# alpc91/SGRL

Measured on AMD Instinct MI355X. Metric: env-steps/sec (whole node) + SET-actor fwd us/step, 3d_walker mix @8192 envs/GPU, higher is better.
Workload: dtype f64 (dynamics) / f32 (SET actor, obs); 1 GPU; 3D_Walker++ 8 variants x 1024 envs per GPU (config 3), random U(-1,1) actions, auto-reset, SET actor forward on every step, random-init weights; envs_per_gpu=8192, obs_max_len=287, action_max_len=21, replay_gather=none (single rank)

## Files before the change

### include/sgrl.h

```cpp
#ifndef SGRL_H
#define SGRL_H

#include <stdint.h>

#ifdef __cplusplus
extern "C" {
#endif

typedef struct sgrl_engine sgrl_engine;

enum {
  SGRL_OK = 0,
  SGRL_ERR_ARG = -1,
  SGRL_ERR_MODEL = -2,
  SGRL_ERR_HIP = -3,
  SGRL_ERR_LIMIT = -4
};

int sgrl_engine_create(int n_morph, const int32_t* const* ib, const int32_t* ib_len, const double* const* fb,
                       const int32_t* fb_len, const int32_t* morph_count, int obs_max_len, int action_max_len,
                       uint64_t seed, uint32_t env_id_base, int max_episode_steps, sgrl_engine** out);
void sgrl_engine_destroy(sgrl_engine* e);

int sgrl_num_envs(const sgrl_engine* e);
int sgrl_record_stride(const sgrl_engine* e);
int sgrl_lds_bytes(const sgrl_engine* e);
int sgrl_launch_groups(const sgrl_engine* e);
int sgrl_fixed_dim_groups(const sgrl_engine* e);
int sgrl_paired_envs(const sgrl_engine* e);

int sgrl_reset(sgrl_engine* e, float* obs, double* obs64, void* stream);

int sgrl_step(sgrl_engine* e, const float* actions, float* obs, float* reward, uint8_t* done, float* dist,
              uint8_t* truncated, double* obs64, double* reward64, int auto_reset, void* stream);

int sgrl_get_records(sgrl_engine* e, double* rec, int32_t* cnt);
int sgrl_set_records(sgrl_engine* e, const double* rec, const int32_t* cnt);
int sgrl_refresh(sgrl_engine* e, float* obs, double* obs64, void* stream);

int sgrl_time_steps(sgrl_engine* e, const float* actions, float* obs, float* reward, uint8_t* done, int reps,
                    void* stream, float* ms_out);

int sgrl_pack_transitions(const float* obs, int ld_obs, const float* action, int ld_act, const float* next_obs, int ld_next,
                          const float* reward, const float* done_f32, const uint8_t* done_u8, const uint8_t* store,
// ... 23 lines not shown
```

### sgrl_amd/_lib.py

```python
import ctypes
import os
import subprocess

_HERE = os.path.dirname(os.path.abspath(__file__))
LIB_PATH = os.environ.get("SGRL_HIP_LIB", os.path.join(_HERE, "libsgrl_hip.so"))
CSRC = os.path.join(_HERE, "csrc")
SOURCES = ["engine.hip", "set_actor.hip", "train_gemm.hip", "render.hip", "swat_actor.hip", "smp_actor.hip"]

_lib = None

_i32p = ctypes.POINTER(ctypes.c_int32)
_f64p = ctypes.POINTER(ctypes.c_double)


class SgrlError(RuntimeError):
    pass


HDR_DIM_FIELDS = (1, 2, 3, 4, 5, 6, 7, 8, 9, 16, 18)
LIGHT_NV = 12
ITAB_GLOBAL = set(x for x in os.environ.get("SGRL_BUILD_ITAB_GLOBAL", "humanoid").split(",") if x and x != "none")
PAIR_NV = {"walker": 15, "hopper": 15}


# ... 44 lines not shown
    hdrs = [os.path.join(CSRC, f) for f in os.listdir(CSRC) if f.endswith((".h", ".inc"))]
    hdrs += [os.path.join(_HERE, "..", "include", f) for f in ("sgrl.h", "sgrl_model.h", "sgrl_set.h", "sgrl_swat.h", "sgrl_smp.h", "sgrl_train.h", "sgrl_render.h")
             if os.path.exists(os.path.join(_HERE, "..", "include", f))]
    newest_hdr = max(os.path.getmtime(d) for d in hdrs)
    objdir = os.path.join(_HERE, "..", "build", "obj")
    os.makedirs(objdir, exist_ok=True)
    base = ["hipcc", "--offload-arch=gfx950", "-O3", "-std=c++17", "-fPIC", "-fno-slp-vectorize"]
    jobs = []
    for sname in SOURCES:
        src = os.path.join(CSRC, sname)
        if os.path.exists(src):
            jobs.append((os.path.join(objdir, sname.replace(".hip", ".o")), src, []))
    spec_src = os.path.join(CSRC, "step_spec.hip")
    for i, w, dims, itab in fams:
        members = ",".join("DimsFixed<%s>" % ",".join(str(x) for x in d) for d in dims)
        flags = ["-DSGRL_SPEC_ID=%d" % i, "-DSGRL_SPEC_WAVES=%d" % w, "-DSGRL_SPEC_FAMILY=" + members]
        if itab:
            flags.append("-DSGRL_ITAB_GLOBAL=1")
        tag = "%08x" % (hash_text(members + str(w) + ("g" if itab else "")) & 0xFFFFFFFF)
        jobs.append((os.path.join(objdir, "family_%d_%s.o" % (i, tag)), spec_src, flags))

    def compile_one(job):
        obj, src, flags = job
        if os.path.exists(obj) and os.path.getmtime(obj) >= max(newest_hdr, os.path.getmtime(src)):
            return False
        cmd = base + flags + ["-c", "-o", obj, src]
        if verbose:
            print(" ".join(cmd), flush=True)
        subprocess.check_call(cmd)
        return True

# ... 19 lines not shown
        raise SgrlError("HIP extension %s is missing: run `python -c 'import __graft_entry__ as g; g.build()'` "
                        "(no CPU fallback exists)" % LIB_PATH)
    import torch
    try:
        L = ctypes.CDLL(LIB_PATH)
    except OSError as e:
        raise SgrlError("cannot load %s: %s" % (LIB_PATH, e))
    L.sgrl_last_error.restype = ctypes.c_char_p
    L.sgrl_version.restype = ctypes.c_char_p
    L.sgrl_engine_create.restype = ctypes.c_int
    L.sgrl_engine_create.argtypes = [ctypes.c_int, ctypes.POINTER(_i32p), _i32p, ctypes.POINTER(_f64p), _i32p, _i32p,
                                     ctypes.c_int, ctypes.c_int, ctypes.c_uint64, ctypes.c_uint32, ctypes.c_int,
                                     ctypes.POINTER(ctypes.c_void_p)]
    L.sgrl_engine_destroy.argtypes = [ctypes.c_void_p]
    L.sgrl_engine_destroy.restype = None
    for name in ("sgrl_num_envs", "sgrl_record_stride", "sgrl_lds_bytes", "sgrl_launch_groups", "sgrl_fixed_dim_groups", "sgrl_paired_envs"):
        getattr(L, name).argtypes = [ctypes.c_void_p]
        getattr(L, name).restype = ctypes.c_int
    vp = ctypes.c_void_p
    L.sgrl_reset.argtypes = [vp, vp, vp, vp]
    L.sgrl_step.argtypes = [vp, vp, vp, vp, vp, vp, vp, vp, vp, ctypes.c_int, vp]
    L.sgrl_refresh.argtypes = [vp, vp, vp, vp]
    L.sgrl_get_records.argtypes = [vp, vp, vp]
    L.sgrl_set_records.argtypes = [vp, vp, vp]
    L.sgrl_time_steps.argtypes = [vp, vp, vp, vp, vp, ctypes.c_int, vp, ctypes.POINTER(ctypes.c_float)]
    ci = ctypes.c_int
    L.sgrl_pack_transitions.argtypes = [vp, ci, vp, ci, vp, ci, vp, vp, vp, vp, vp, vp, ci, ci, ci, vp]
    L.sgrl_ingest_rows.argtypes = [vp, ci, ci, ci, vp, vp, ci, vp]
    L.sgrl_ingest_block.argtypes = [vp, ci, ci, ci, vp, ci, vp, vp, vp, vp, vp]
    L.sgrl_round_record.argtypes = [vp, vp, vp, vp, vp, vp, vp, vp, vp, ci, ci, vp]
    L.sgrl_ingest_ws_words.argtypes = [ci]
    L.sgrl_ingest_ws_words.restype = ctypes.c_int64
    _lib = L
    return L


EXPORTS = ["sgrl_engine_create", "sgrl_engine_destroy", "sgrl_num_envs", "sgrl_record_stride", "sgrl_lds_bytes", "sgrl_launch_groups", "sgrl_fixed_dim_groups", "sgrl_paired_envs",
           "sgrl_reset", "sgrl_step", "sgrl_get_records", "sgrl_set_records", "sgrl_refresh", "sgrl_time_steps", "sgrl_pack_transitions", "sgrl_round_record", "sgrl_ingest_rows", "sgrl_ingest_block", "sgrl_ingest_ws_words",
           "sgrl_last_error", "sgrl_version"]


def check(rc, what):
    if rc != 0:
        raise SgrlError("%s failed (%d): %s" % (what, rc, lib().sgrl_last_error().decode()))
```

### sgrl_amd/csrc/engine.hip

```cpp
#include <hip/hip_runtime.h>

#include <algorithm>
#include <cstdio>
#include <cstdlib>
#include <cstring>
#include <string>
#include <vector>

#include "engine_kernel.h"
#include "stream_pick.h"

namespace {

thread_local std::string g_err;

int fail(int code, const std::string& msg) {
  g_err = msg;
  return code;
}
#define HIP_TRY(expr)                                                                              \
  do {                                                                                             \
    hipError_t _e = (expr);                                                                        \
    if (_e != hipSuccess)                                                                          \
      return fail(SGRL_ERR_HIP, std::string(#expr) + ": " + hipGetErrorString(_e));                \
// ... 18 lines not shown
  sgrl::HipWave w;
  const sgrl::StepIO io = make_io(a, out, env);
  sgrl::env_reset(w, m, o, S, I, io, true);
}

__global__ __launch_bounds__(64) void k_env_refresh(BatchArgs a, StepOut out) {
  const int env = __builtin_amdgcn_readfirstlane(a.block_env[blockIdx.x]);
  SgrlModelView m; sgrl::Layout o; double* S; int32_t* I;
  setup<DimsAny>(a, env, &m, &o, &S, &I);
  sgrl::HipWave w;
  const sgrl::StepIO io = make_io(a, out, env);
  sgrl::env_refresh(w, m, o, S, I, io);
}

typedef int (*SpecLaunch)(int, int, void*, const void*, const void*);
struct SpecFamily { int waves; int n; SpecLaunch launch; int itab_global; };
struct SpecMember { int family, slot; int dims[12]; };
}
#ifndef SGRL_NO_SPECS
#define SGRL_FAMILY(id, waves, n, itab) extern "C" int sgrl_spec_launch_##id(int, int, void*, const void*, const void*);
#define SGRL_MEMBER(...)
#include "spec_table.inc"
#undef SGRL_FAMILY
#undef SGRL_MEMBER
namespace {
const SpecFamily kFamilies[] = {
#define SGRL_FAMILY(id, waves, n, itab) {waves, n, sgrl_spec_launch_##id, itab},
#define SGRL_MEMBER(...)
#include "spec_table.inc"
#undef SGRL_FAMILY
#undef SGRL_MEMBER
};
const SpecMember kMembers[] = {
#define SGRL_FAMILY(id, waves, n, itab)
#define SGRL_MEMBER(fam, slot, ...) {fam, slot, {__VA_ARGS__}},
#include "spec_table.inc"
#undef SGRL_FAMILY
#undef SGRL_MEMBER
};
constexpr int kNumMembers = (int)(sizeof(kMembers) / sizeof(kMembers[0]));
}
#else
namespace {
const SpecFamily kFamilies[1] = {{0, 0, nullptr, 0}};
const SpecMember kMembers[1] = {{-1, -1, {0}}};
constexpr int kNumMembers = 0;
}
#endif
namespace {
int spec_for(const int32_t* hdr, int waves) {
  static const int fields[11] = {SGRL_H_NBODY, SGRL_H_NJNT, SGRL_H_NQ, SGRL_H_NV, SGRL_H_NU, SGRL_H_NGEOM, SGRL_H_NPAIR,
                                 SGRL_H_INTEGRATOR, SGRL_H_FRAME_SKIP, SGRL_H_MAX_ROWS, SGRL_H_SOLVER};
  for (int k = 0; k < kNumMembers; k++) {
    if (kFamilies[kMembers[k].family].waves != waves) continue;
    bool same = true;
    for (int f = 0; f < 11 && same; f++) same = kMembers[k].dims[f] == hdr[fields[f]];
    if (same) return k;
  }
  return -1;
}
}

struct sgrl_engine {
  int n_morph = 0, n_env = 0, stride = 0, lds_bytes = 0, scratch_stride = 0;
  int obs_max_len = 0, action_max_len = 0;
  std::vector<int32_t*> d_ib;
  std::vector<double*> d_fb;
  MorphDev* d_morphs = nullptr;
  int32_t* d_env_morph = nullptr;
  int32_t* d_block_env = nullptr;
  int32_t* d_step_env = nullptr;
  int32_t* d_step_mate = nullptr;
  int n_paired = 0;
  double* d_rec = nullptr;
  int32_t* d_cnt = nullptr;
  double* d_scratch = nullptr;
  BatchArgs args{};
  struct Group {
    int first = 0, count = 0, lds = 0; bool light = false; int spec = -1; hipStream_t stream = nullptr; hipEvent_t done = nullptr;
    int step_first = 0, step_count = 0, step_lds = 0;
  };
  std::vector<Group> groups;
  bool groups_checked = false;
  hipEvent_t fork = nullptr;
  std::vector<int> morph_lds;
};

namespace {
template <class K>
int launch_groups(sgrl_engine* e, K kernel_in, const StepOut& out, hipStream_t user, bool is_step = false) {
  auto pick = [&](const sgrl_engine::Group& g) { return (is_step && g.light) ? k_env_step_light : kernel_in; };
  auto launch = [&](const sgrl_engine::Group& g, const BatchArgs& a_in, hipStream_t st) -> int {
    const BatchArgs& a = a_in;
    if (is_step && g.spec >= 0) {
      BatchArgs b = a_in;
      b.block_env = e->d_step_env + g.step_first;
      b.block_mate = e->d_step_mate + g.step_first;
      const int rc = kFamilies[g.spec].launch(g.step_count, g.step_lds, st, &b, &out);
      return rc == 0 ? SGRL_OK : fail(SGRL_ERR_HIP, std::string("fixed-dimension step kernel launch failed: ") + hipGetErrorString((hipError_t)rc));
    }
    hipLaunchKernelGGL(pick(g), dim3(g.count), dim3(64), g.lds, st, a, out);
    return SGRL_OK;
  };
  if (e->groups.size() == 1) {
    const int rc = launch(e->groups[0], e->args, user);
    if (rc != SGRL_OK) return rc;
  } else {
    if (!e->groups_checked && sgrl_streams::enabled()) {
      hipStreamCaptureStatus cap = hipStreamCaptureStatusNone;
      (void)hipStreamIsCapturing(user, &cap);
      if (cap == hipStreamCaptureStatusNone) {
        std::vector<hipStream_t> taken;
        for (auto& g : e->groups) {
// ... 185 lines not shown
  if (host && hipMemcpyFromSymbol(host, HIP_SYMBOL(sgrl_engine_dev::g_phase_prof), sizeof(unsigned long long) * 16 * (size_t)n_env) != hipSuccess) return -2;
  if (reset) { static unsigned long long z[16 * 65536]; if (hipMemcpyToSymbol(HIP_SYMBOL(sgrl_engine_dev::g_phase_prof), z, sizeof(z)) != hipSuccess) return -3; }
  return 0;
}
#endif

void sgrl_engine_destroy(sgrl_engine* e) {
  if (!e) return;
  for (auto p : e->d_ib) if (p) (void)hipFree(p);
  for (auto p : e->d_fb) if (p) (void)hipFree(p);
  if (e->d_morphs) (void)hipFree(e->d_morphs);
  if (e->d_env_morph) (void)hipFree(e->d_env_morph);
  if (e->d_block_env) (void)hipFree(e->d_block_env);
  if (e->d_step_env) (void)hipFree(e->d_step_env);
  if (e->d_step_mate) (void)hipFree(e->d_step_mate);
  if (e->d_rec) (void)hipFree(e->d_rec);
  if (e->d_cnt) (void)hipFree(e->d_cnt);
  if (e->d_scratch) (void)hipFree(e->d_scratch);
  for (auto& g : e->groups) { if (g.stream) (void)hipStreamDestroy(g.stream); if (g.done) (void)hipEventDestroy(g.done); }
  if (e->fork) (void)hipEventDestroy(e->fork);
  delete e;
}

int sgrl_engine_create(int n_morph, const int32_t* const* ib, const int32_t* ib_len, const double* const* fb,
                       const int32_t* fb_len, const int32_t* morph_count, int obs_max_len, int action_max_len,
                       uint64_t seed, uint32_t env_id_base, int max_episode_steps, sgrl_engine** out) {
  if (!out) return fail(SGRL_ERR_ARG, "out is null");
  *out = nullptr;
  if (n_morph <= 0 || !ib || !ib_len || !fb || !fb_len || !morph_count) return fail(SGRL_ERR_ARG, "null or empty morphology list");
  int ndev = 0;
// ... 141 lines not shown
            e->n_paired += 2;
            i += 2;
          } else {
            step_env.push_back(order[i]); step_mate.push_back(-1);
            i++;
          }
        }
        if (const char* pad = getenv("SGRL_LDS_PAD")) { g.lds += atoi(pad); g.step_lds += atoi(pad); e->lds_bytes = std::max(e->lds_bytes, g.lds); }
        g.count = i - g.first;
        g.step_count = (int)step_env.size() - g.step_first;
        e->lds_bytes = std::max(e->lds_bytes, std::max(g.step_lds, g.lds));
        e->groups.push_back(g);
      }
      (void)hipMemcpy(e->d_step_env, step_env.data(), sizeof(int32_t) * step_env.size(), hipMemcpyHostToDevice);
      (void)hipMemcpy(e->d_step_mate, step_mate.data(), sizeof(int32_t) * step_mate.size(), hipMemcpyHostToDevice);
    } else {
      std::vector<int> cost(n_morph), cls(n_morph);
      bool light_batch = true;
      for (int k = 0; k < n_morph; k++) {
        cost[k] = ib[k][SGRL_H_NV];
        const int granule = 1280;
        int per_cu = (160 * 1024) / (((e->morph_lds[k] + granule - 1) / granule) * granule);
        cls[k] = per_cu > 8 ? 8 : per_cu;
        light_batch = light_batch && ib[k][SGRL_H_NV] <= kLightNv && per_cu >= kLightPerCu;
      }
      if (light_batch) for (int k = 0; k < n_morph; k++) cls[k] = kLightPerCu;
      std::stable_sort(order.begin(), order.end(), [&](int32_t x, int32_t y) {
        const int mx = env_morph[x], my = env_morph[y];
        if (cls[mx] != cls[my]) return cls[mx] < cls[my];
        return cost[mx] > cost[my];
// ... 54 lines not shown
  BatchArgs& a = e->args;
  a.morphs = e->d_morphs; a.env_morph = e->d_env_morph; a.block_env = e->d_block_env; a.rec = e->d_rec; a.cnt = e->d_cnt; a.scratch = e->d_scratch;
  a.scratch_stride = e->scratch_stride;
  a.stride = e->stride; a.n_env = e->n_env; a.obs_max_len = obs_max_len; a.action_max_len = action_max_len;
  a.seed = seed; a.env_id_base = env_id_base; a.max_episode_steps = max_episode_steps;
  if (hipDeviceSynchronize() != hipSuccess) { sgrl_engine_destroy(e); return fail(SGRL_ERR_HIP, "device error during engine setup"); }
  *out = e;
  return SGRL_OK;
}

int sgrl_num_envs(const sgrl_engine* e) { return e ? e->n_env : SGRL_ERR_ARG; }
int sgrl_record_stride(const sgrl_engine* e) { return e ? e->stride : SGRL_ERR_ARG; }
int sgrl_lds_bytes(const sgrl_engine* e) { return e ? e->lds_bytes : SGRL_ERR_ARG; }
int sgrl_launch_groups(const sgrl_engine* e) { return e ? (int)e->groups.size() : SGRL_ERR_ARG; }
int sgrl_paired_envs(const sgrl_engine* e) { return e ? e->n_paired : SGRL_ERR_ARG; }
int sgrl_fixed_dim_groups(const sgrl_engine* e) {
  if (!e) return SGRL_ERR_ARG;
  int n = 0;
  for (const auto& g : e->groups) n += g.spec >= 0 ? 1 : 0;
  return n;
}

int sgrl_reset(sgrl_engine* e, float* obs, double* obs64, void* stream) {
  if (!e || !obs) return fail(SGRL_ERR_ARG, "sgrl_reset: null engine or obs");
  StepOut out{};
  out.obs32 = obs; out.obs64 = obs64;
  return launch_groups(e, k_env_reset, out, (hipStream_t)stream);
}

int sgrl_step(sgrl_engine* e, const float* actions, float* obs, float* reward, uint8_t* done, float* dist,
// ... 112 lines not shown
```

### sgrl_amd/csrc/engine_kernel.h

```cpp
#pragma once
#include <hip/hip_runtime.h>

#include <stdint.h>

#ifndef SGRL_ITAB_GLOBAL
#define SGRL_ITAB_GLOBAL 0
#endif
#ifndef SGRL_STAGE_FLOATS
#define SGRL_STAGE_FLOATS 0
#endif
#if defined(__HIP_DEVICE_COMPILE__)
#define SGRL_CONST_AS __attribute__((address_space(4)))
#if SGRL_ITAB_GLOBAL
#define SGRL_ITAB_AS __attribute__((address_space(4)))
#else
#define SGRL_ITAB_AS __attribute__((address_space(3)))
#endif
#if SGRL_STAGE_FLOATS
#define SGRL_FTAB_AS __attribute__((address_space(3)))
#else
#define SGRL_FTAB_AS __attribute__((address_space(4)))
#endif
#endif
#include "../../include/sgrl.h"
// ... 6 lines not shown
using sgrl::DimsAny;
using sgrl::DimsFixed;

struct MorphDev {
  const int32_t* ib;
  const double* fb;
  int32_t slot;
  int32_t pad_;
};

struct BatchArgs {
  const MorphDev* morphs;
  const int32_t* env_morph;
  const int32_t* block_env;
  const int32_t* block_mate;
  double* rec;
  int32_t* cnt;
  double* scratch;
  int scratch_stride;
  int stride;
  int n_env;
  int obs_max_len, action_max_len;
  uint64_t seed;
  uint32_t env_id_base;
  int max_episode_steps;
};

struct StepOut {
  const float* actions;
  float* obs32;
  double* obs64;
  float* reward;
  double* reward64;
  uint8_t* done;
  float* dist;
  uint8_t* truncated;
  int auto_reset;
};


#ifdef SGRL_PHASE_PROF
__device__ unsigned long long g_phase_prof[16 * 65536];
__device__ __forceinline__ unsigned long long* sgrl_phase_prof_buf() { return g_phase_prof; }
#endif

extern __shared__ double sgrl_lds[];

template <class D>
__device__ __forceinline__ void setup(const BatchArgs& a, int env, SgrlModelView* m, sgrl::Layout* o, double** S, int32_t** I) {
  const int mi = __builtin_amdgcn_readfirstlane(a.env_morph[env]);
  const MorphDev md = a.morphs[mi];
  int32_t hdr[SGRL_NHDR];
#pragma unroll
  for (int k = 0; k < SGRL_NHDR; k++) hdr[k] = __builtin_amdgcn_readfirstlane(md.ib[k]);
  D::apply(hdr);
  int n_int, n_f64;
  sgrl_model_blob_sizes(hdr, &n_int, &n_f64);
  sgrl::make_layout(hdr, o, (D::kFixed && SGRL_ITAB_GLOBAL) ? 0 : n_int, SGRL_STAGE_FLOATS ? n_f64 : 0);
  double* s = sgrl_lds;
  int32_t* ii = reinterpret_cast<int32_t*>(sgrl_lds + o->s_total);
  const int lane = threadIdx.x;
  if (SGRL_STAGE_FLOATS) for (int k = lane; k < n_f64; k += 64) s[o->model_f + k] = md.fb[k];
#if !SGRL_ITAB_GLOBAL
  for (int k = lane; k < n_int; k += 64) ii[o->model_i + k] = md.ib[k];
#endif
  __syncthreads();
#if SGRL_STAGE_FLOATS
  sgrl_ftab_t ftab = (sgrl_ftab_t)(s + o->model_f);
#else
  sgrl_ftab_t ftab = (sgrl_ftab_t)md.fb;
#endif
#if SGRL_ITAB_GLOBAL
  sgrl_model_view_dims(hdr, (sgrl_hdr_t)md.ib, (sgrl_fhdr_t)md.fb, (sgrl_itab_t)md.ib, ftab, m);
#else
  sgrl_model_view_dims(hdr, (sgrl_hdr_t)md.ib, (sgrl_fhdr_t)md.fb, (sgrl_itab_t)(ii + o->model_i), ftab, m);
#endif
  *S = s;
  *I = ii;
}

__device__ __forceinline__ sgrl::StepIO make_io(const BatchArgs& a, const StepOut& out, int env) {
  sgrl::StepIO io;
  io.rec = a.rec + (size_t)env * a.stride;
  io.cnt = a.cnt + (size_t)env * 4;
  io.action = out.actions ? out.actions + (size_t)env * a.action_max_len : nullptr;
  io.obs32 = out.obs32 ? out.obs32 + (size_t)env * a.obs_max_len : nullptr;
  io.obs64 = out.obs64 ? out.obs64 + (size_t)env * a.obs_max_len : nullptr;
  io.reward = out.reward ? out.reward + env : nullptr;
  io.reward64 = out.reward64 ? out.reward64 + env : nullptr;
  io.done = out.done ? out.done + env : nullptr;
  io.dist = out.dist ? out.dist + env : nullptr;
  io.truncated = out.truncated ? out.truncated + env : nullptr;
  io.obs_max_len = a.obs_max_len;
// ... 10 lines not shown
__device__ __forceinline__ void env_step_wave(const BatchArgs& a, const StepOut& out, int env) {
  SgrlModelView m; sgrl::Layout o; double* S; int32_t* I;
  setup<D>(a, env, &m, &o, &S, &I);
  W w;
#ifdef SGRL_PHASE_PROF
  w.prof = sgrl_phase_prof_buf() + 16 * (size_t)(env & 65535);
  const long long t_begin = __builtin_readcyclecounter();
#endif
  const sgrl::StepIO io = make_io(a, out, env);
  sgrl::env_step(w, m, o, S, I, io);
#ifdef SGRL_PHASE_PROF
  if (w.lane == 0) w.prof[15] += (unsigned long long)(__builtin_readcyclecounter() - t_begin);
#endif
}

template <class D, class W>
__device__ __forceinline__ void env_step_pair(const BatchArgs& a, const StepOut& out, int env_a, int env_b) {
  static_assert(!SGRL_STAGE_FLOATS && !SGRL_ITAB_GLOBAL, "the pair layout shares the LDS copy of the int tables only");
  const int mi = __builtin_amdgcn_readfirstlane(a.env_morph[env_a]);
  const MorphDev md = a.morphs[mi];
  int32_t hdr[SGRL_NHDR];
#pragma unroll
  for (int k = 0; k < SGRL_NHDR; k++) hdr[k] = __builtin_amdgcn_readfirstlane(md.ib[k]);
  D::apply(hdr);
  int n_int, n_f64;
  sgrl_model_blob_sizes(hdr, &n_int, &n_f64);
  sgrl::Layout o;
  sgrl::make_layout(hdr, &o, n_int, 0, true);
  int32_t* const ia = reinterpret_cast<int32_t*>(sgrl_lds + o.s_total);
  for (int k = threadIdx.x; k < n_int; k += 64) ia[o.model_i + k] = md.ib[k];
  __syncthreads();
  SgrlModelView m;
  sgrl_model_view_dims(hdr, (sgrl_hdr_t)md.ib, (sgrl_fhdr_t)md.fb, (sgrl_itab_t)(ia + o.model_i), (sgrl_ftab_t)md.fb, &m);
  W w;
  double* const S = sgrl_lds + w.half * o.pair_stride;
  int32_t* const I = ia + 2 * w.half * o.pair_stride;
  const sgrl::StepIO io = make_io(a, out, w.half ? env_b : env_a);
  sgrl::env_step(w, m, o, S, I, io);
}

template <int I, class... Ds> struct FamilyRun {
  __device__ static __forceinline__ void run(int, int, int, const BatchArgs&, const StepOut&) {}
};
template <int I, class D, class... Rest> struct FamilyRun<I, D, Rest...> {
  __device__ static __forceinline__ void run(int slot, int env, int mate, const BatchArgs& a, const StepOut& out) {
    if (slot == I) {
      if constexpr (D::kPair) {
        if (mate >= 0) { env_step_pair<D, sgrl::HalfWaveT<D::kNv, sgrl::HipHalfPrim<D>>>(a, out, env, mate); return; }
      }
      env_step_wave<D, sgrl::HipWaveT<(D::kNv <= 24 ? D::kNv : 24), D>>(a, out, env);
      return;
    }
    FamilyRun<I + 1, Rest...>::run(slot, env, mate, a, out);
  }
};

}
```

### sgrl_amd/csrc/step_spec.hip

```cpp
#include "engine_kernel.h"

#ifndef SGRL_SPEC_ID
#error "compile with -DSGRL_SPEC_ID=<k> -DSGRL_SPEC_WAVES=<w> -DSGRL_SPEC_FAMILY=DimsFixed<...>,..."
#endif
#define SGRL_CAT2(a, b) a##b
#define SGRL_CAT(a, b) SGRL_CAT2(a, b)

namespace {
using namespace sgrl_engine_dev;

__global__ __launch_bounds__(64) __attribute__((amdgpu_waves_per_eu(SGRL_SPEC_WAVES, SGRL_SPEC_WAVES))) void k_env_step_spec(BatchArgs a, StepOut out) {
  const int env = __builtin_amdgcn_readfirstlane(a.block_env[blockIdx.x]);
  const int mate = __builtin_amdgcn_readfirstlane(a.block_mate[blockIdx.x]);
  const int slot = __builtin_amdgcn_readfirstlane(a.morphs[__builtin_amdgcn_readfirstlane(a.env_morph[env])].slot);
  FamilyRun<0, SGRL_SPEC_FAMILY>::run(slot, env, mate, a, out);
}
}

extern "C" int SGRL_CAT(sgrl_spec_launch_, SGRL_SPEC_ID)(int n_wg, int lds, void* stream, const void* batch_args, const void* step_out) {
  static int lds_limit[64];
  static bool init = false;
  if (!init) { for (int& v : lds_limit) v = 48 * 1024; init = true; }
  int dev = 0;
  (void)hipGetDevice(&dev);
  int& limit = lds_limit[dev >= 0 && dev < 64 ? dev : 0];
  if (lds > limit) {
    const hipError_t e = hipFuncSetAttribute(reinterpret_cast<const void*>(k_env_step_spec), hipFuncAttributeMaxDynamicSharedMemorySize, lds);
    if (e != hipSuccess) return (int)e;
    limit = lds;
  }
  hipLaunchKernelGGL(k_env_step_spec, dim3(n_wg), dim3(64), lds, (hipStream_t)stream, *reinterpret_cast<const BatchArgs*>(batch_args),
                     *reinterpret_cast<const StepOut*>(step_out));
  return (int)hipGetLastError();
}
```

### sgrl_amd/vec_env.py

```python
import collections.abc
import ctypes

import numpy as np

from . import _lib, mjcf, model_pack
from .env_spec import env_spec_for


class Box(object):

    def __init__(self, low, high, shape=None, dtype=np.float32):
        if shape is None:
            shape = np.shape(low)
        self.low = np.full(shape, low, dtype=dtype) if np.isscalar(low) else np.asarray(low, dtype=dtype)
        self.high = np.full(shape, high, dtype=dtype) if np.isscalar(high) else np.asarray(high, dtype=dtype)
        self.shape = tuple(shape)
        self.dtype = np.dtype(dtype)

    def sample(self):
        return np.random.uniform(self.low, self.high).astype(self.dtype)


class StepInfos(collections.abc.Sequence):
    __slots__ = ("_dist", "_trunc", "_extra")
# ... 95 lines not shown
        fbp = (ctypes.POINTER(ctypes.c_double) * k)(*[b[1].ctypes.data_as(ctypes.POINTER(ctypes.c_double)) for b in self._blobs])
        ibl = (ctypes.c_int32 * k)(*[len(b[0]) for b in self._blobs])
        fbl = (ctypes.c_int32 * k)(*[len(b[1]) for b in self._blobs])
        cnt = (ctypes.c_int32 * k)(*self.counts)
        h = ctypes.c_void_p()
        _lib.check(L.sgrl_engine_create(k, ibp, ibl, fbp, fbl, cnt, self.obs_max_len, self.action_max_len,
                                        ctypes.c_uint64(int(seed)), ctypes.c_uint32(int(env_id_base)),
                                        int(max_episode_steps), ctypes.byref(h)), "sgrl_engine_create")
        self._h = h
        self._L = L
        self.stride = L.sgrl_record_stride(h)
        self.lds_bytes = L.sgrl_lds_bytes(h)
        self.launch_groups = L.sgrl_launch_groups(h)
        self.fixed_dim_groups = L.sgrl_fixed_dim_groups(h)
        self.paired_envs = L.sgrl_paired_envs(h)
        dev = self.device
        secs = [("obs", 4 * n * self.obs_max_len), ("rew", 4 * n), ("dist", 4 * n), ("done", n), ("trunc", n)]
        self._out_off, off = {}, 0
        for name, nbytes in secs:
            self._out_off[name] = (off, nbytes)
            off += _round_up(nbytes)
        self._out = torch.zeros(off, dtype=torch.uint8, device=dev)
        sec = lambda name: self._out[self._out_off[name][0]:self._out_off[name][0] + self._out_off[name][1]]
        self.obs = sec("obs").view(torch.float32).view(n, self.obs_max_len)
        self.rew = sec("rew").view(torch.float32)
        self.dist = sec("dist").view(torch.float32)
        self.done = sec("done")
        self.trunc = sec("trunc")
        self._act = torch.zeros((n, self.action_max_len), dtype=torch.float32, device=dev)
        self._act_host = None
# ... 162 lines not shown
```

Measured before the change: 1.960 million env-steps/s.

## Use persistent workgroups with cost-balanced static job schedule for fixed-dim step kernels

Replaces one-workgroup-per-env launches of the specialized step kernel with a persistent grid sized to occupancy times CU count. A host-side LPT greedy scheduler assigns jobs by per-morphology cycle cost to slots, grouping same-morphology jobs so staged LDS tables are reused across consecutive envs. This aims to cut tail imbalance and repeated table staging. It also disables machine LICM for these kernels to limit register pressure, and it adds a hardcoded cost table plus optional profiling stamps.

```diff
diff --git a/include/sgrl.h b/include/sgrl.h
--- a/include/sgrl.h
+++ b/include/sgrl.h
@@ -28,6 +28,8 @@
 int sgrl_launch_groups(const sgrl_engine* e);
 int sgrl_fixed_dim_groups(const sgrl_engine* e);
 int sgrl_paired_envs(const sgrl_engine* e);
+int sgrl_step_workgroups(const sgrl_engine* e);
+int sgrl_plan_step_schedule(int n_jobs, const int32_t* cost, const int32_t* key, int slots, int32_t* off, int32_t* job);
 
 int sgrl_reset(sgrl_engine* e, float* obs, double* obs64, void* stream);
 
diff --git a/sgrl_amd/_lib.py b/sgrl_amd/_lib.py
--- a/sgrl_amd/_lib.py
+++ b/sgrl_amd/_lib.py
@@ -82,7 +82,7 @@
     spec_src = os.path.join(CSRC, "step_spec.hip")
     for i, w, dims, itab in fams:
         members = ",".join("DimsFixed<%s>" % ",".join(str(x) for x in d) for d in dims)
-        flags = ["-DSGRL_SPEC_ID=%d" % i, "-DSGRL_SPEC_WAVES=%d" % w, "-DSGRL_SPEC_FAMILY=" + members]
+        flags = ["-DSGRL_SPEC_ID=%d" % i, "-DSGRL_SPEC_WAVES=%d" % w, "-DSGRL_SPEC_FAMILY=" + members, "-mllvm", "-disable-machine-licm"]
         if itab:
             flags.append("-DSGRL_ITAB_GLOBAL=1")
         tag = "%08x" % (hash_text(members + str(w) + ("g" if itab else "")) & 0xFFFFFFFF)
@@ -132,10 +132,11 @@
                                      ctypes.POINTER(ctypes.c_void_p)]
     L.sgrl_engine_destroy.argtypes = [ctypes.c_void_p]
     L.sgrl_engine_destroy.restype = None
-    for name in ("sgrl_num_envs", "sgrl_record_stride", "sgrl_lds_bytes", "sgrl_launch_groups", "sgrl_fixed_dim_groups", "sgrl_paired_envs"):
+    for name in ("sgrl_num_envs", "sgrl_record_stride", "sgrl_lds_bytes", "sgrl_launch_groups", "sgrl_fixed_dim_groups", "sgrl_paired_envs", "sgrl_step_workgroups"):
         getattr(L, name).argtypes = [ctypes.c_void_p]
         getattr(L, name).restype = ctypes.c_int
     vp = ctypes.c_void_p
+    L.sgrl_plan_step_schedule.argtypes = [ctypes.c_int, _i32p, _i32p, ctypes.c_int, _i32p, _i32p]
     L.sgrl_reset.argtypes = [vp, vp, vp, vp]
     L.sgrl_step.argtypes = [vp, vp, vp, vp, vp, vp, vp, vp, vp, ctypes.c_int, vp]
     L.sgrl_refresh.argtypes = [vp, vp, vp, vp]
@@ -153,7 +154,7 @@
     return L
 
 
-EXPORTS = ["sgrl_engine_create", "sgrl_engine_destroy", "sgrl_num_envs", "sgrl_record_stride", "sgrl_lds_bytes", "sgrl_launch_groups", "sgrl_fixed_dim_groups", "sgrl_paired_envs",
+EXPORTS = ["sgrl_engine_create", "sgrl_engine_destroy", "sgrl_num_envs", "sgrl_record_stride", "sgrl_lds_bytes", "sgrl_launch_groups", "sgrl_fixed_dim_groups", "sgrl_paired_envs", "sgrl_step_workgroups", "sgrl_plan_step_schedule",
            "sgrl_reset", "sgrl_step", "sgrl_get_records", "sgrl_set_records", "sgrl_refresh", "sgrl_time_steps", "sgrl_pack_transitions", "sgrl_round_record", "sgrl_ingest_rows", "sgrl_ingest_block", "sgrl_ingest_ws_words",
            "sgrl_last_error", "sgrl_version"]
 
diff --git a/sgrl_amd/csrc/engine.hip b/sgrl_amd/csrc/engine.hip
--- a/sgrl_amd/csrc/engine.hip
+++ b/sgrl_amd/csrc/engine.hip
@@ -4,6 +4,7 @@
 #include <cstdio>
 #include <cstdlib>
 #include <cstring>
+#include <queue>
 #include <string>
 #include <vector>
 
@@ -56,18 +57,21 @@
 }
 
 typedef int (*SpecLaunch)(int, int, void*, const void*, const void*);
-struct SpecFamily { int waves; int n; SpecLaunch launch; int itab_global; };
+typedef int (*SpecOccupancy)(int);
+struct SpecFamily { int waves; int n; SpecLaunch launch; SpecOccupancy occupancy; int itab_global; };
 struct SpecMember { int family, slot; int dims[12]; };
 }
 #ifndef SGRL_NO_SPECS
-#define SGRL_FAMILY(id, waves, n, itab) extern "C" int sgrl_spec_launch_##id(int, int, void*, const void*, const void*);
+#define SGRL_FAMILY(id, waves, n, itab)                                             \
+  extern "C" int sgrl_spec_launch_##id(int, int, void*, const void*, const void*); \
+  extern "C" int sgrl_spec_occupancy_##id(int);
 #define SGRL_MEMBER(...)
 #include "spec_table.inc"
 #undef SGRL_FAMILY
 #undef SGRL_MEMBER
 namespace {
 const SpecFamily kFamilies[] = {
-#define SGRL_FAMILY(id, waves, n, itab) {waves, n, sgrl_spec_launch_##id, itab},
+#define SGRL_FAMILY(id, waves, n, itab) {waves, n, sgrl_spec_launch_##id, sgrl_spec_occupancy_##id, itab},
 #define SGRL_MEMBER(...)
 #include "spec_table.inc"
 #undef SGRL_FAMILY
@@ -84,7 +88,7 @@
 }
 #else
 namespace {
-const SpecFamily kFamilies[1] = {{0, 0, nullptr, 0}};
+const SpecFamily kFamilies[1] = {{0, 0, nullptr, nullptr, 0}};
 const SpecMember kMembers[1] = {{-1, -1, {0}}};
 constexpr int kNumMembers = 0;
 }
@@ -101,6 +105,57 @@
   }
   return -1;
 }
+
+void plan_step_schedule(int n_jobs, const int32_t* cost, const int32_t* key, int slots, int32_t* off, int32_t* job) {
+  std::vector<int32_t> by_cost(n_jobs);
+  for (int j = 0; j < n_jobs; j++) by_cost[j] = j;
+  auto heavier = [&](int32_t x, int32_t y) { return cost[x] != cost[y] ? cost[x] > cost[y] : (key[x] != key[y] ? key[x] < key[y] : x < y); };
+  std::sort(by_cost.begin(), by_cost.end(), heavier);
+  typedef std::pair<long long, int> Load;
+  std::priority_queue<Load, std::vector<Load>, std::greater<Load>> heap;
+  for (int l = 0; l < slots; l++) heap.push(Load(0, l));
+  std::vector<std::vector<int32_t>> lists(slots);
+  std::vector<long long> load(slots, 0);
+  for (int32_t j : by_cost) {
+    const Load top = heap.top();
+    heap.pop();
+    lists[top.second].push_back(j);
+    load[top.second] += cost[j];
+    heap.push(Load(load[top.second], top.second));
+  }
+  std::vector<int> by_load(slots);
+  for (int l = 0; l < slots; l++) by_load[l] = l;
+  std::stable_sort(by_load.begin(), by_load.end(), [&](int x, int y) { return load[x] > load[y]; });
+  std::vector<int> list_of(slots);
+  for (int r = 0; r < slots; r++) {
+    const int row = r / 8, col = r % 8, width = std::min(8, slots - 8 * row);
+    list_of[8 * row + ((row & 1) ? width - 1 - col : col)] = by_load[r];
+  }
+  int n = 0;
+  for (int w = 0; w < slots; w++) {
+    off[w] = n;
+    const std::vector<int32_t>& l = lists[list_of[w]];
+    std::vector<char> taken(l.size(), 0);
+    for (size_t i = 0; i < l.size(); i++) {
+      if (taken[i]) continue;
+      job[n++] = ~l[i];
+      for (size_t k = i + 1; k < l.size(); k++)
+        if (!taken[k] && key[l[k]] == key[l[i]]) { job[n++] = l[k]; taken[k] = 1; }
+    }
+  }
+  off[slots] = n;
+}
+
+struct StepCost { int nbody, nv, pair, kcycles; };
+const StepCost kStepCost[] = {
+  {3, 9, 0, 1090},  {3, 9, 1, 1200},  {4, 12, 0, 1220}, {4, 12, 1, 1415}, {5, 15, 0, 1390}, {5, 15, 1, 1610},
+  {6, 18, 0, 1620}, {7, 21, 0, 2010}, {8, 24, 0, 1920},
+};
+int step_job_cost(const int32_t* hdr, bool pair) {
+  for (const StepCost& c : kStepCost)
+    if (c.nbody == hdr[SGRL_H_NBODY] && c.nv == hdr[SGRL_H_NV] && c.pair == (pair ? 1 : 0)) return c.kcycles;
+  return (600 + 60 * hdr[SGRL_H_NV]) * (pair ? 23 : 20) / 20;
+}
 }
 
 struct sgrl_engine {
@@ -113,6 +168,13 @@
   int32_t* d_block_env = nullptr;
   int32_t* d_step_env = nullptr;
   int32_t* d_step_mate = nullptr;
+  int32_t* d_sched_off = nullptr;
+  int32_t* d_sched_job = nullptr;
+  int step_slots = 0;
+#ifdef SGRL_PHASE_PROF
+  unsigned long long* d_job_prof = nullptr;
+  std::vector<int32_t> h_step_env, h_step_mate;
+#endif
   int n_paired = 0;
   double* d_rec = nullptr;
   int32_t* d_cnt = nullptr;
@@ -121,6 +183,7 @@
   struct Group {
     int first = 0, count = 0, lds = 0; bool light = false; int spec = -1; hipStream_t stream = nullptr; hipEvent_t done = nullptr;
     int step_first = 0, step_count = 0, step_lds = 0;
+    int sched_first = 0, sched_wg = 0;
   };
   std::vector<Group> groups;
   bool groups_checked = false;
@@ -138,7 +201,12 @@
       BatchArgs b = a_in;
       b.block_env = e->d_step_env + g.step_first;
       b.block_mate = e->d_step_mate + g.step_first;
-      const int rc = kFamilies[g.spec].launch(g.step_count, g.step_lds, st, &b, &out);
+      b.sched_off = e->d_sched_off + g.sched_first;
+      b.sched_job = e->d_sched_job + g.step_first;
+#ifdef SGRL_PHASE_PROF
+      b.job_prof = e->d_job_prof + 4 * (size_t)g.step_first;
+#endif
+      const int rc = kFamilies[g.spec].launch(g.sched_wg, g.step_lds, st, &b, &out);
       return rc == 0 ? SGRL_OK : fail(SGRL_ERR_HIP, std::string("fixed-dimension step kernel launch failed: ") + hipGetErrorString((hipError_t)rc));
     }
     hipLaunchKernelGGL(pick(g), dim3(g.count), dim3(64), g.lds, st, a, out);
@@ -354,6 +422,11 @@
   if (e->d_block_env) (void)hipFree(e->d_block_env);
   if (e->d_step_env) (void)hipFree(e->d_step_env);
   if (e->d_step_mate) (void)hipFree(e->d_step_mate);
+  if (e->d_sched_off) (void)hipFree(e->d_sched_off);
+  if (e->d_sched_job) (void)hipFree(e->d_sched_job);
+#ifdef SGRL_PHASE_PROF
+  if (e->d_job_prof) (void)hipFree(e->d_job_prof);
+#endif
   if (e->d_rec) (void)hipFree(e->d_rec);
   if (e->d_cnt) (void)hipFree(e->d_cnt);
   if (e->d_scratch) (void)hipFree(e->d_scratch);
@@ -525,6 +598,49 @@
       }
       (void)hipMemcpy(e->d_step_env, step_env.data(), sizeof(int32_t) * step_env.size(), hipMemcpyHostToDevice);
       (void)hipMemcpy(e->d_step_mate, step_mate.data(), sizeof(int32_t) * step_mate.size(), hipMemcpyHostToDevice);
+      const char* ss = getenv("SGRL_STEP_SCHED");
+      const bool persistent = !(ss && ss[0] == '0');
+      int n_cu = 0;
+      {
+        int dev = 0;
+        (void)hipGetDevice(&dev);
+        (void)hipDeviceGetAttribute(&n_cu, hipDeviceAttributeMultiprocessorCount, dev);
+      }
+      std::vector<int32_t> sched_off, sched_job(step_env.size());
+      for (auto& g : e->groups) {
+        int per_cu = kFamilies[g.spec].occupancy(g.step_lds);
+        const int by_lds = sgrl::workgroups_per_cu(g.step_lds);
+        if (per_cu <= 0 || per_cu > by_lds) per_cu = by_lds;
+        const int slots = std::max(1, per_cu * std::max(1, n_cu));
+        g.sched_first = (int)sched_off.size();
+        g.sched_wg = persistent ? std::min(slots, g.step_count) : g.step_count;
+        sched_off.resize(sched_off.size() + g.sched_wg + 1);
+        std::vector<int32_t> cost(g.step_count), key(g.step_count);
+        for (int j = 0; j < g.step_count; j++) {
+          const int k = env_morph[step_env[g.step_first + j]];
+          const bool pair = step_mate[g.step_first + j] >= 0;
+          cost[j] = step_job_cost(ib[k], pair);
+          key[j] = 2 * k + (pair ? 1 : 0);
+        }
+        if (persistent) {
+          plan_step_schedule(g.step_count, cost.data(), key.data(), g.sched_wg, sched_off.data() + g.sched_first, sched_job.data() + g.step_first);
+        } else {
+          for (int j = 0; j < g.step_count; j++) { sched_off[g.sched_first + j] = j; sched_job[g.step_first + j] = ~j; }
+          sched_off[g.sched_first + g.step_count] = g.step_count;
+        }
+        e->step_slots += g.sched_wg;
+      }
+      if (hipMalloc(&e->d_sched_off, sizeof(int32_t) * sched_off.size()) != hipSuccess || hipMalloc(&e->d_sched_job, sizeof(int32_t) * sched_job.size()) != hipSuccess) {
+        sgrl_engine_destroy(e);
+        return fail(SGRL_ERR_HIP, "hipMalloc(step schedule) failed");
+      }
+      (void)hipMemcpy(e->d_sched_off, sched_off.data(), sizeof(int32_t) * sched_off.size(), hipMemcpyHostToDevice);
+      (void)hipMemcpy(e->d_sched_job, sched_job.data(), sizeof(int32_t) * sched_job.size(), hipMemcpyHostToDevice);
+#ifdef SGRL_PHASE_PROF
+      e->h_step_env = step_env; e->h_step_mate = step_mate;
+      if (hipMalloc(&e->d_job_prof, 32 * step_env.size()) != hipSuccess) { sgrl_engine_destroy(e); return fail(SGRL_ERR_HIP, "hipMalloc(job stamps) failed"); }
+      (void)hipMemset(e->d_job_prof, 0, 32 * step_env.size());
+#endif
     } else {
       std::vector<int> cost(n_morph), cls(n_morph);
       bool light_batch = true;
@@ -609,6 +725,30 @@
 int sgrl_lds_bytes(const sgrl_engine* e) { return e ? e->lds_bytes : SGRL_ERR_ARG; }
 int sgrl_launch_groups(const sgrl_engine* e) { return e ? (int)e->groups.size() : SGRL_ERR_ARG; }
 int sgrl_paired_envs(const sgrl_engine* e) { return e ? e->n_paired : SGRL_ERR_ARG; }
+int sgrl_step_workgroups(const sgrl_engine* e) { return e ? e->step_slots : SGRL_ERR_ARG; }
+int sgrl_plan_step_schedule(int n_jobs, const int32_t* cost, const int32_t* key, int slots, int32_t* off, int32_t* job) {
+  if (n_jobs < 0 || slots <= 0 || !off || (n_jobs > 0 && (!cost || !key || !job))) return fail(SGRL_ERR_ARG, "sgrl_plan_step_schedule: bad argument");
+  for (int j = 0; j < n_jobs; j++) if (cost[j] <= 0) return fail(SGRL_ERR_ARG, "sgrl_plan_step_schedule: a job's cost must be positive");
+  plan_step_schedule(n_jobs, cost, key, slots, off, job);
+  return SGRL_OK;
+}
+#ifdef SGRL_PHASE_PROF
+int sgrl_job_prof(sgrl_engine* e, unsigned long long* host, int reset) {
+  if (!e || !e->d_job_prof || hipDeviceSynchronize() != hipSuccess) return -1;
+  const size_t n = e->h_step_env.size();
+  if (host) {
+    std::vector<unsigned long long> t(4 * n);
+    if (hipMemcpy(t.data(), e->d_job_prof, 32 * n, hipMemcpyDeviceToHost) != hipSuccess) return -2;
+    for (size_t j = 0; j < n; j++) {
+      for (int k = 0; k < 4; k++) host[6 * j + k] = t[4 * j + k];
+      host[6 * j + 4] = (unsigned long long)(long long)e->h_step_env[j];
+      host[6 * j + 5] = (unsigned long long)(long long)e->h_step_mate[j];
+    }
+  }
+  if (reset && hipMemset(e->d_job_prof, 0, 32 * n) != hipSuccess) return -3;
+  return (int)n;
+}
+#endif
 int sgrl_fixed_dim_groups(const sgrl_engine* e) {
   if (!e) return SGRL_ERR_ARG;
   int n = 0;
diff --git a/sgrl_amd/csrc/engine_kernel.h b/sgrl_amd/csrc/engine_kernel.h
--- a/sgrl_amd/csrc/engine_kernel.h
+++ b/sgrl_amd/csrc/engine_kernel.h
@@ -44,6 +44,8 @@
   const int32_t* env_morph;
   const int32_t* block_env;
   const int32_t* block_mate;
+  const int32_t* sched_off;
+  const int32_t* sched_job;
   double* rec;
   int32_t* cnt;
   double* scratch;
@@ -54,6 +56,9 @@
   uint64_t seed;
   uint32_t env_id_base;
   int max_episode_steps;
+#ifdef SGRL_PHASE_PROF
+  unsigned long long* job_prof;
+#endif
 };
 
 struct StepOut {
@@ -76,37 +81,50 @@
 
 extern __shared__ double sgrl_lds[];
 
+struct Staged {
+  MorphDev md;
+  int32_t hdr[SGRL_NHDR];
+};
+template <class D, bool PAIR>
+__device__ __forceinline__ void staged_layout(const int32_t* hdr, sgrl::Layout* o, int* n_int, int* n_f64) {
+  sgrl_model_blob_sizes(hdr, n_int, n_f64);
+  if (PAIR) sgrl::make_layout(hdr, o, *n_int, 0, true);
+  else sgrl::make_layout(hdr, o, (D::kFixed && SGRL_ITAB_GLOBAL) ? 0 : *n_int, SGRL_STAGE_FLOATS ? *n_f64 : 0);
+}
+template <class D, bool PAIR>
+__device__ __forceinline__ void stage_tables(const BatchArgs& a, int env, Staged* st) {
+  const int mi = __builtin_amdgcn_readfirstlane(a.env_morph[env]);
+  st->md = a.morphs[mi];
+#pragma unroll
+  for (int k = 0; k < SGRL_NHDR; k++) st->hdr[k] = __builtin_amdgcn_readfirstlane(st->md.ib[k]);
+  D::apply(st->hdr);
+  sgrl::Layout o;
+  int n_int, n_f64;
+  staged_layout<D, PAIR>(st->hdr, &o, &n_int, &n_f64);
+  double* s = sgrl_lds;
+  int32_t* ii = reinterpret_cast<int32_t*>(sgrl_lds + o.s_total);
+  const int lane = threadIdx.x;
+  if (SGRL_STAGE_FLOATS && !PAIR) for (int k = lane; k < n_f64; k += 64) s[o.model_f + k] = st->md.fb[k];
+  if (PAIR || !SGRL_ITAB_GLOBAL) for (int k = lane; k < n_int; k += 64) ii[o.model_i + k] = st->md.ib[k];
+  __syncthreads();
+}
+template <class D, bool PAIR>
+__device__ __forceinline__ void view_tables(const Staged& st, SgrlModelView* m, sgrl::Layout* o, double** S, int32_t** I) {
+  int n_int, n_f64;
+  staged_layout<D, PAIR>(st.hdr, o, &n_int, &n_f64);
+  double* s = sgrl_lds;
+  int32_t* ii = reinterpret_cast<int32_t*>(sgrl_lds + o->s_total);
+  sgrl_ftab_t ftab = (SGRL_STAGE_FLOATS && !PAIR) ? (sgrl_ftab_t)(s + o->model_f) : (sgrl_ftab_t)st.md.fb;
+  sgrl_itab_t itab = (SGRL_ITAB_GLOBAL && !PAIR) ? (sgrl_itab_t)st.md.ib : (sgrl_itab_t)(ii + o->model_i);
+  sgrl_model_view_dims(st.hdr, (sgrl_hdr_t)st.md.ib, (sgrl_fhdr_t)st.md.fb, itab, ftab, m);
+  *S = s;
+  *I = ii;
+}
 template <class D>
 __device__ __forceinline__ void setup(const BatchArgs& a, int env, SgrlModelView* m, sgrl::Layout* o, double** S, int32_t** I) {
-  const int mi = __builtin_amdgcn_readfirstlane(a.env_morph[env]);
-  const MorphDev md = a.morphs[mi];
-  int32_t hdr[SGRL_NHDR];
-#pragma unroll
-  for (int k = 0; k < SGRL_NHDR; k++) hdr[k] = __builtin_amdgcn_readfirstlane(md.ib[k]);
-  D::apply(hdr);
-  int n_int, n_f64;
-  sgrl_model_blob_sizes(hdr, &n_int, &n_f64);
-  sgrl::make_layout(hdr, o, (D::kFixed && SGRL_ITAB_GLOBAL) ? 0 : n_int, SGRL_STAGE_FLOATS ? n_f64 : 0);
-  double* s = sgrl_lds;
-  int32_t* ii = reinterpret_cast<int32_t*>(sgrl_lds + o->s_total);
-  const int lane = threadIdx.x;
-  if (SGRL_STAGE_FLOATS) for (int k = lane; k < n_f64; k += 64) s[o->model_f + k] = md.fb[k];
-#if !SGRL_ITAB_GLOBAL
-  for (int k = lane; k < n_int; k += 64) ii[o->model_i + k] = md.ib[k];
-#endif
-  __syncthreads();
-#if SGRL_STAGE_FLOATS
-  sgrl_ftab_t ftab = (sgrl_ftab_t)(s + o->model_f);
-#else
-  sgrl_ftab_t ftab = (sgrl_ftab_t)md.fb;
-#endif
-#if SGRL_ITAB_GLOBAL
-  sgrl_model_view_dims(hdr, (sgrl_hdr_t)md.ib, (sgrl_fhdr_t)md.fb, (sgrl_itab_t)md.ib, ftab, m);
-#else
-  sgrl_model_view_dims(hdr, (sgrl_hdr_t)md.ib, (sgrl_fhdr_t)md.fb, (sgrl_itab_t)(ii + o->model_i), ftab, m);
-#endif
-  *S = s;
-  *I = ii;
+  Staged st;
+  stage_tables<D, false>(a, env, &st);
+  view_tables<D, false>(st, m, o, S, I);
 }
 
 __device__ __forceinline__ sgrl::StepIO make_io(const BatchArgs& a, const StepOut& out, int env) {
@@ -147,45 +165,96 @@
 #endif
 }
 
-template <class D, class W>
-__device__ __forceinline__ void env_step_pair(const BatchArgs& a, const StepOut& out, int env_a, int env_b) {
-  static_assert(!SGRL_STAGE_FLOATS && !SGRL_ITAB_GLOBAL, "the pair layout shares the LDS copy of the int tables only");
-  const int mi = __builtin_amdgcn_readfirstlane(a.env_morph[env_a]);
-  const MorphDev md = a.morphs[mi];
-  int32_t hdr[SGRL_NHDR];
-#pragma unroll
-  for (int k = 0; k < SGRL_NHDR; k++) hdr[k] = __builtin_amdgcn_readfirstlane(md.ib[k]);
-  D::apply(hdr);
-  int n_int, n_f64;
-  sgrl_model_blob_sizes(hdr, &n_int, &n_f64);
-  sgrl::Layout o;
-  sgrl::make_layout(hdr, &o, n_int, 0, true);
-  int32_t* const ia = reinterpret_cast<int32_t*>(sgrl_lds + o.s_total);
-  for (int k = threadIdx.x; k < n_int; k += 64) ia[o.model_i + k] = md.ib[k];
-  __syncthreads();
-  SgrlModelView m;
-  sgrl_model_view_dims(hdr, (sgrl_hdr_t)md.ib, (sgrl_fhdr_t)md.fb, (sgrl_itab_t)(ia + o.model_i), (sgrl_ftab_t)md.fb, &m);
-  W w;
-  double* const S = sgrl_lds + w.half * o.pair_stride;
-  int32_t* const I = ia + 2 * w.half * o.pair_stride;
-  const sgrl::StepIO io = make_io(a, out, w.half ? env_b : env_a);
-  sgrl::env_step(w, m, o, S, I, io);
+#ifdef SGRL_PHASE_PROF
+__device__ __forceinline__ unsigned long long sgrl_wave_place() {
+  const unsigned hw = __builtin_amdgcn_s_getreg((31 << 11) | 4), xcc = __builtin_amdgcn_s_getreg((31 << 11) | 20);
+  return ((unsigned long long)xcc << 32) | hw;
+}
+struct JobStamp {
+  unsigned long long* p; unsigned long long t0; long long c0;
+  __device__ __forceinline__ JobStamp(const BatchArgs& a, int job) : p(a.job_prof ? a.job_prof + 4 * (size_t)job : nullptr), t0(wall_clock64()), c0(__builtin_readcyclecounter()) {}
+  __device__ __forceinline__ void done() {
+    if (p && threadIdx.x == 0) { p[0] = t0; p[1] = wall_clock64(); p[2] += (unsigned long long)(__builtin_readcyclecounter() - c0); p[3] = sgrl_wave_place(); }
+  }
+};
+#define SGRL_JOB_BEGIN(a, job) JobStamp job_stamp(a, job)
+#define SGRL_JOB_END() job_stamp.done()
+#else
+#define SGRL_JOB_BEGIN(a, job)
+#define SGRL_JOB_END()
+#endif
+
+struct StepArgs { BatchArgs a; StepOut out; };
+__device__ __forceinline__ void step_args(BatchArgs* a, StepOut* out) {
+  const char SGRL_CONST_AS* p = (const char SGRL_CONST_AS*)__builtin_amdgcn_kernarg_segment_ptr();
+  __builtin_memcpy(a, p + __builtin_offsetof(StepArgs, a), sizeof(BatchArgs));
+  __builtin_memcpy(out, p + __builtin_offsetof(StepArgs, out), sizeof(StepOut));
+}
+
+template <class T> __device__ __forceinline__ T* opaque_uniform(T* p) {
+  const unsigned long long v = (unsigned long long)p;
+  unsigned lo = __builtin_amdgcn_readfirstlane((unsigned)v), hi = __builtin_amdgcn_readfirstlane((unsigned)(v >> 32));
+  asm volatile("" : "+s"(lo), "+s"(hi));
+  return (T*)(((unsigned long long)hi << 32) | lo);
+}
+
+template <class D, class W, bool PAIR>
+__device__ __forceinline__ int env_step_run(int job, int j, int end) {
+  static_assert(!PAIR || (!SGRL_STAGE_FLOATS && !SGRL_ITAB_GLOBAL), "the pair layout shares the LDS copy of the int tables only");
+  Staged st;
+  {
+    BatchArgs a; StepOut out;
+    step_args(&a, &out);
+    stage_tables<D, PAIR>(a, __builtin_amdgcn_readfirstlane(a.block_env[job]), &st);
+  }
+  for (;;) {
+    BatchArgs a; StepOut out;
+    step_args(&a, &out);
+    st.md.ib = opaque_uniform(st.md.ib);
+    st.md.fb = opaque_uniform(st.md.fb);
+    SgrlModelView m; sgrl::Layout o; double* S; int32_t* I;
+    view_tables<D, PAIR>(st, &m, &o, &S, &I);
+    SGRL_JOB_BEGIN(a, job);
+    {
+      W w;
+      w.fence_lane();
+      int env = __builtin_amdgcn_readfirstlane(a.block_env[job]);
+      if constexpr (PAIR) {
+        asm volatile("" : "+v"(w.half));
+        const int env_b = __builtin_amdgcn_readfirstlane(a.block_mate[job]);
+        env = w.half ? env_b : env;
+        S += w.half * o.pair_stride;
+        I += 2 * w.half * o.pair_stride;
+      } else {
+#ifdef SGRL_PHASE_PROF
+        w.prof = sgrl_phase_prof_buf() + 16 * (size_t)(env & 65535);
+#endif
+      }
+      const sgrl::StepIO io = make_io(a, out, env);
+      sgrl::env_step(w, m, o, S, I, io);
+    }
+    SGRL_JOB_END();
+    if (++j >= end) return j;
+    step_args(&a, &out);
+    job = __builtin_amdgcn_readfirstlane(a.sched_job[j]);
+    if (job < 0) return j;
+    __syncthreads();
+  }
 }
 
 template <int I, class... Ds> struct FamilyRun {
-  __device__ static __forceinline__ void run(int, int, int, const BatchArgs&, const StepOut&) {}
+  __device__ static __forceinline__ int run(int, int, bool, int, int end) { return end; }
 };
 template <int I, class D, class... Rest> struct FamilyRun<I, D, Rest...> {
-  __device__ static __forceinline__ void run(int slot, int env, int mate, const BatchArgs& a, const StepOut& out) {
+  __device__ static __forceinline__ int run(int slot, int job, bool pair, int j, int end) {
     if (slot == I) {
       if constexpr (D::kPair) {
-        if (mate >= 0) { env_step_pair<D, sgrl::HalfWaveT<D::kNv, sgrl::HipHalfPrim<D>>>(a, out, env, mate); return; }
+        if (pair) return env_step_run<D, sgrl::HalfWaveT<D::kNv, sgrl::HipHalfPrim<D>>, true>(job, j, end);
       }
-      env_step_wave<D, sgrl::HipWaveT<(D::kNv <= 24 ? D::kNv : 24), D>>(a, out, env);
-      return;
+      return env_step_run<D, sgrl::HipWaveT<(D::kNv <= 24 ? D::kNv : 24), D>, false>(job, j, end);
     }
-    FamilyRun<I + 1, Rest...>::run(slot, env, mate, a, out);
-  }
-};
-
-}
+    return FamilyRun<I + 1, Rest...>::run(slot, job, pair, j, end);
+  }
+};
+
+}
diff --git a/sgrl_amd/csrc/step_spec.hip b/sgrl_amd/csrc/step_spec.hip
--- a/sgrl_amd/csrc/step_spec.hip
+++ b/sgrl_amd/csrc/step_spec.hip
@@ -9,12 +9,31 @@
 namespace {
 using namespace sgrl_engine_dev;
 
-__global__ __launch_bounds__(64) __attribute__((amdgpu_waves_per_eu(SGRL_SPEC_WAVES, SGRL_SPEC_WAVES))) void k_env_step_spec(BatchArgs a, StepOut out) {
-  const int env = __builtin_amdgcn_readfirstlane(a.block_env[blockIdx.x]);
-  const int mate = __builtin_amdgcn_readfirstlane(a.block_mate[blockIdx.x]);
-  const int slot = __builtin_amdgcn_readfirstlane(a.morphs[__builtin_amdgcn_readfirstlane(a.env_morph[env])].slot);
-  FamilyRun<0, SGRL_SPEC_FAMILY>::run(slot, env, mate, a, out);
+__global__ __launch_bounds__(64) __attribute__((amdgpu_waves_per_eu(SGRL_SPEC_WAVES, SGRL_SPEC_WAVES))) void k_env_step_spec(StepArgs) {
+  int j, end;
+  {
+    BatchArgs a; StepOut out;
+    step_args(&a, &out);
+    j = __builtin_amdgcn_readfirstlane(a.sched_off[blockIdx.x]);
+    end = __builtin_amdgcn_readfirstlane(a.sched_off[blockIdx.x + 1]);
+  }
+  while (j < end) {
+    BatchArgs a; StepOut out;
+    step_args(&a, &out);
+    const int job = ~__builtin_amdgcn_readfirstlane(a.sched_job[j]);
+    const int env = __builtin_amdgcn_readfirstlane(a.block_env[job]);
+    const bool pair = __builtin_amdgcn_readfirstlane(a.block_mate[job]) >= 0;
+    const int slot = __builtin_amdgcn_readfirstlane(a.morphs[__builtin_amdgcn_readfirstlane(a.env_morph[env])].slot);
+    j = FamilyRun<0, SGRL_SPEC_FAMILY>::run(slot, job, pair, j, end);
+    if (j < end) __syncthreads();
+  }
 }
+}
+
+extern "C" int SGRL_CAT(sgrl_spec_occupancy_, SGRL_SPEC_ID)(int lds) {
+  int n = 0;
+  const hipError_t e = hipOccupancyMaxActiveBlocksPerMultiprocessor(&n, k_env_step_spec, 64, (size_t)lds);
+  return e == hipSuccess ? n : -(int)e;
 }
 
 extern "C" int SGRL_CAT(sgrl_spec_launch_, SGRL_SPEC_ID)(int n_wg, int lds, void* stream, const void* batch_args, const void* step_out) {
@@ -29,7 +48,7 @@
     if (e != hipSuccess) return (int)e;
     limit = lds;
   }
-  hipLaunchKernelGGL(k_env_step_spec, dim3(n_wg), dim3(64), lds, (hipStream_t)stream, *reinterpret_cast<const BatchArgs*>(batch_args),
-                     *reinterpret_cast<const StepOut*>(step_out));
+  const StepArgs ka{*reinterpret_cast<const BatchArgs*>(batch_args), *reinterpret_cast<const StepOut*>(step_out)};
+  hipLaunchKernelGGL(k_env_step_spec, dim3(n_wg), dim3(64), lds, (hipStream_t)stream, ka);
   return (int)hipGetLastError();
 }
diff --git a/sgrl_amd/vec_env.py b/sgrl_amd/vec_env.py
--- a/sgrl_amd/vec_env.py
+++ b/sgrl_amd/vec_env.py
@@ -133,6 +133,7 @@
         self.launch_groups = L.sgrl_launch_groups(h)
         self.fixed_dim_groups = L.sgrl_fixed_dim_groups(h)
         self.paired_envs = L.sgrl_paired_envs(h)
+        self.step_workgroups = L.sgrl_step_workgroups(h)
         dev = self.device
         secs = [("obs", 4 * n * self.obs_max_len), ("rew", 4 * n), ("dist", 4 * n), ("done", n), ("trunc", n)]
         self._out_off, off = {}, 0
```

Measured after the change: 1.815 million env-steps/s. 7.4% lower.
